# apache/incubator-predictionio

Measured on NVIDIA H100. Metric: ALS iterations/sec, higher is better.
Workload: dtype f32

## Files before the change

### incubator-predictionio_b200/csrc/als_pair_kernel.cuh

```cuda
#pragma once
#include <cuda_fp16.h>
#include <cuda_runtime.h>
#include <stdint.h>

#include "als_kernels.cuh"
#include "als_lockstep.cuh"

namespace pio {
namespace pr {

constexpr int KP = 64;
constexpr int CH = 8;
constexpr int RSTR = KP;
constexpr int NSTAGE = 4;
constexpr int STAGE = CH * RSTR;
constexpr int NTILE = 20;
using LL = LsLayout<KP>;
constexpr int SLOT_STRIDE = LL::STRIDE;
constexpr int VSTR = 80;
constexpr int PART_FLOATS = LL::SIZE + KP;
static_assert(NSTAGE * STAGE <= SLOT_STRIDE, "the staging ring lives in the second slot");
static_assert(NSTAGE % 2 == 0, "a loop step consumes two stages");
constexpr int W_BVEC = 2 * SLOT_STRIDE;
constexpr int W_COL = W_BVEC + 2 * VSTR;
// ... 137 lines not shown
#pragma unroll
    for (int i = 0; i < 4; ++i) {
#pragma unroll
      for (int e = 0; e < 2; ++e) {
        const int q = 2 * i + e;
        const int c0 = xo[q & 3] + 32 * (q >> 2), c4 = 4 * RSTR + xo[q & 3] + 32 * (1 - (q >> 2));
        const float a0 = XA[c0], a4 = XA[c4], b0 = XB[c0], b4 = XB[c4];
        pb[i][e] = fmaf(wb[0], a0, pb[i][e]);
        pb[i][e] = fmaf(wb[1], a4, pb[i][e]);
        pb[i][e] = fmaf(wb[2], b0, pb[i][e]);
        pb[i][e] = fmaf(wb[3], b4, pb[i][e]);
        split2(__fmul_rn(a0, sc[0]), __fmul_rn(a4, sc[1]), hi[i][e], lo[i][e]);
        split2(__fmul_rn(b0, sc[2]), __fmul_rn(b4, sc[3]), hi[i][e + 2], lo[i][e + 2]);
      }
    }
#pragma unroll
    for (int j = 0; j < 8; ++j) {
      const int bi = j >> 1, be = j & 1;
      const uint64_t bh = pack2(hi[bi][be], hi[bi][be + 2]), bl = pack2(lo[bi][be], lo[bi][be + 2]);
#pragma unroll
      for (int i = bi; i < 4; ++i) {
        const int tile = i * (i + 1) + j;
        float d[4];
        mma_f16_zp(d, lo[i], bh);
        mma_f16_p(d, hi[i], bl);
        mma_f16_p(d, hi[i], bh);
        acc[tile][0] += d[0];
        acc[tile][1] += d[1];
        acc[tile][2] += d[2];
        acc[tile][3] += d[3];
      }
    }
  }
  cp_async_wait<0>();
  __syncwarp();

#pragma unroll
  for (int i = 0; i < 4; ++i)
#pragma unroll
    for (int e = 0; e < 2; ++e) {
      float v = pb[i][e];
      v += __shfl_xor_sync(0xffffffffu, v, 1);
      v += __shfl_xor_sync(0xffffffffu, v, 2);
      if (t == 0) bv[16 * i + 8 * e + g] = v;
    }
  {
    const float* yl = yty ? yty + g * KP + 2 * t : nullptr;
    int tile = 0;
#pragma unroll
    for (int i = 0; i < 4; ++i) {
#pragma unroll
      for (int j = 0; j <= 2 * i + 1; ++j, ++tile) {
        const int cb = j >> 1;
        const int cc = 8 * (j & 1) + 2 * t;
        float d0 = acc[tile][0] * unscale, d1 = acc[tile][1] * unscale;
        float d2 = acc[tile][2] * unscale, d3 = acc[tile][3] * unscale;
        if (yl) {
          const float2 y0 = __ldg(reinterpret_cast<const float2*>(yl + 16 * i * KP + 8 * j));
          const float2 y1 = __ldg(reinterpret_cast<const float2*>(yl + (16 * i + 8) * KP + 8 * j));
          d0 += y0.x; d1 += y0.y;
          d2 += y1.x; d3 += y1.y;
        }
        if (cb < i) {
          *reinterpret_cast<float2*>(slot + LL::offd(i, cb, g, cc)) = make_float2(d0, d1);
          *reinterpret_cast<float2*>(slot + LL::offd(i, cb, g + 8, cc)) = make_float2(d2, d3);
        } else {
          if (cc <= g) slot[LL::diag(i, g, cc)] = d0;
          if (cc + 1 <= g) slot[LL::diag(i, g, cc + 1)] = d1;
          if (cc <= g + 8) slot[LL::diag(i, g + 8, cc)] = d2;
          if (cc + 1 <= g + 8) slot[LL::diag(i, g + 8, cc + 1)] = d3;
        }
      }
    }
  }
  __syncwarp();
}

__device__ __forceinline__ void fill_identity(float* slot, float* bv) {
  const int lane = threadIdx.x & 31;
  for (int o = lane; o < LL::SIZE; o += 32) slot[o] = 0.f;
  __syncwarp();
  for (int r = lane; r < KP; r += 32) {
    slot[LL::at(r, r)] = 1.f;
    bv[r] = 0.f;
  }
  __syncwarp();
}

template <bool IMPLICIT, int WARPS>
__global__ void __launch_bounds__(32 * WARPS, 12 / WARPS) als_solve_pair_kernel(const SolveParams p, int n_items) {
  extern __shared__ __align__(16) float smem_all[];
  const int warp = threadIdx.x >> 5;
  float* smem = smem_all + warp * W_FLOATS;
  float* slot0 = smem;
  float* slot1 = smem + SLOT_STRIDE;
  float* ring = slot1;
  float* bvec = smem + W_BVEC;
  float* colbuf = smem + W_COL;
  float* mval = smem + W_MVAL;
  const int lane = threadIdx.x & 31;
  const int grp = lane >> 4;
  const int npairs = (n_items + 1) >> 1;
  const float c1_root_max = IMPLICIT ? sqrtf(p.alpha * __uint_as_float(__ldg(p.absmax + 1))) : 1.f;
  const int e = split_exponent(__uint_as_float(__ldg(p.absmax)) * c1_root_max);
  const float s = pow2f(e), unscale = pow2f(-2 * e);

#pragma unroll 1
  for (int base = blockIdx.x * WARPS; base < npairs; base += gridDim.x * WARPS) {
    const int pair = base + warp;
    int row0 = -1, row1 = -1;
    if (pair < npairs) {
#pragma unroll 1
      for (int h = 0; h < 2; ++h) {
        const int item = 2 * pair + h;
        float* slot = h ? slot1 : slot0;
        float* bv = bvec + h * VSTR;
        if (item >= n_items) {
          fill_identity(slot, bv);
          continue;
        }
        long long beg, end;
        if (p.partial) {
          beg = p.wl_beg[item];
          end = p.wl_end[item];
        } else {
          const int r = p.row_begin + item;
          beg = p.ptr[r];
          end = p.ptr[r + 1];
          if (h) row1 = r;
          else row0 = r;
        }
        accumulate_row<IMPLICIT>(p, beg, end, s, unscale, IMPLICIT && !p.partial ? p.yty : nullptr, ring, mval, slot, bv);
        if (p.partial) {
          float* out = p.partial + (size_t)item * PART_FLOATS;
          for (int o = lane; o < LL::SIZE / 4; o += 32)
            reinterpret_cast<float4*>(out)[o] = reinterpret_cast<const float4*>(slot)[o];
          for (int o = lane; o < KP; o += 32) out[LL::SIZE + o] = bv[o];
          __syncwarp();
        }
      }
    }
    if (p.partial) continue;
    if (WARPS > 1) __syncthreads();
    if (pair < npairs) {
      const int myrow = grp ? row1 : row0;
      const int rr = myrow < 0 ? p.row_begin : myrow;
      chol_lockstep<KP>(grp ? slot1 : slot0, bvec + grp * VSTR, p.lambda * p.nreg[rr], p.k, colbuf + grp * VSTR,
                        p.dst + (size_t)(p.dst_row_offset + rr) * KP, myrow >= 0, p.fail);
      __syncwarp();
    }
  }
}

template <bool IMPLICIT>
__global__ void __launch_bounds__(32, 12) als_finish_pair_kernel(const SolveParams p, const int* __restrict__ row_part_ptr,
                                                                  int n_rows) {
  extern __shared__ __align__(16) float smem[];
  float* bvec = smem + W_BVEC;
  float* colbuf = smem + W_COL;
  const int lane = threadIdx.x & 31;
  const int grp = lane >> 4;
  const int npairs = (n_rows + 1) >> 1;
#pragma unroll 1
  for (int pair = blockIdx.x; pair < npairs; pair += gridDim.x) {
#pragma unroll 1
    for (int h = 0; h < 2; ++h) {
      const int r = 2 * pair + h;
      float* slot = smem + h * SLOT_STRIDE;
      float* bv = bvec + h * VSTR;
      if (r >= n_rows) {
        fill_identity(slot, bv);
        continue;
      }
      const int p0 = row_part_ptr[r], p1 = row_part_ptr[r + 1];
      for (int o = lane; o < PART_FLOATS / 4; o += 32) {
        float4 s = make_float4(0.f, 0.f, 0.f, 0.f);
        for (int q = p0; q < p1; ++q) {
          const float4 v = __ldg(reinterpret_cast<const float4*>(p.partial + (size_t)q * PART_FLOATS) + o);
          s.x += v.x; s.y += v.y; s.z += v.z; s.w += v.w;
        }
        if (o < LL::SIZE / 4) reinterpret_cast<float4*>(slot)[o] = s;
        else reinterpret_cast<float4*>(bv)[o - LL::SIZE / 4] = s;
      }
      __syncwarp();
      if (IMPLICIT) {
        ls_add_yty<KP>(slot, p.yty);
        __syncwarp();
      }
    }
    const int myrow = 2 * pair + grp;
    const bool valid = myrow < n_rows;
    const int rr = valid ? myrow : 0;
    chol_lockstep<KP>(smem + grp * SLOT_STRIDE, bvec + grp * VSTR, p.lambda * p.nreg[rr], p.k, colbuf + grp * VSTR,
                      p.dst + (size_t)(p.dst_row_offset + rr) * KP, valid, p.fail);
    __syncwarp();
  }
}

}
}
```

### incubator-predictionio_b200/csrc/pio_als.cu

```cuda
#include "../../include/pio_als.h"

#include <cuda_runtime.h>
#include <dlfcn.h>
#include <math.h>
#include <nccl.h>
#include <stdarg.h>
#include <stdio.h>
#include <stdlib.h>
#include <string.h>

#include <chrono>
#include <algorithm>
#include <array>
#include <deque>
#include <exception>
#include <map>
#include <memory>
#include <mutex>
#include <string>
#include <type_traits>
#include <vector>

#include "als_kernels.cuh"
#include "als_mma_kernel.cuh"
// ... 196 lines not shown
}
__global__ void extract_csr_kernel(const uint64_t* keys, const uint32_t* pay, const float* rating, long long b,
                                   long long cnt, int bits_col, const int* p2i_col, int* idx, float* val) {
  const long long t = (long long)blockIdx.x * blockDim.x + threadIdx.x;
  if (t >= cnt) return;
  idx[t] = p2i_col[(int)(keys[b + t] & ((1ull << bits_col) - 1ull))];
  val[t] = rating[pay[b + t]];
}
__global__ void local_rows_kernel(const long long* ptr_full, int row0, int R, long long base, const int* inv,
                                  const uint32_t* deg, const uint32_t* npos, int implicit, long long* ptr,
                                  float* nreg, int* counts , int heavy_t) {
  const int r = blockIdx.x * blockDim.x + threadIdx.x;
  if (r > R) return;
  ptr[r] = ptr_full[row0 + r] - base;
  if (r == R) return;
  const int ext = inv[row0 + r];
  float nr = 0.f;
  if (ext >= 0) {
    const uint32_t d = deg[ext];
    nr = implicit ? (float)npos[ext] : (float)d;
    if (d > 0) atomicAdd(&counts[0], 1);
    if (d > (uint32_t)heavy_t) atomicAdd(&counts[1], 1);
  }
  nreg[r] = nr;
}
__global__ void scatter_init_kernel(const float* ext_f, int n, int k, int kp, const int* perm, const uint32_t* deg,
                                    float* F) {
  const long long o = (long long)blockIdx.x * blockDim.x + threadIdx.x;
  if (o >= (long long)n * kp) return;
  const int r = (int)(o / kp), c = (int)(o % kp);
  float v = 0.f;
  if (c < k && deg[r] > 0) v = ext_f[(size_t)r * k + c];
  F[(size_t)perm[r] * kp + c] = v;
}
__device__ __forceinline__ uint64_t splitmix64_dev(uint64_t x) {
  x += 0x9E3779B97F4A7C15ull;
  uint64_t z = x;
  z = (z ^ (z >> 30)) * 0xBF58476D1CE4E5B9ull;
  z = (z ^ (z >> 27)) * 0x94D049BB133111EBull;
  return z ^ (z >> 31);
}
__global__ void hash_init_kernel(int n, int k, int kp, uint64_t seed, int side, const int* perm,
                                 const uint32_t* deg, float* F) {
  const int r = blockIdx.x * blockDim.x + threadIdx.x;
  if (r >= n) return;
  float* row = F + (size_t)perm[r] * kp;
  if (deg[r] == 0) {
    for (int c = 0; c < kp; ++c) row[c] = 0.f;
    return;
  }
  const uint64_t s = seed ^ 0xA5A5A5A55A5A5A5Aull;
  double nrm = 0.0;
  for (int c = 0; c < k; ++c) {
    const uint64_t ctr = ((uint64_t)r * (uint64_t)k + (uint64_t)c) * 2ull + ((uint64_t)side << 62);
    const uint64_t h1 = splitmix64_dev(s ^ ctr), h2 = splitmix64_dev(s ^ (ctr + 1ull));
    const double u1 = ((double)(h1 >> 11) + 1.0) * (1.0 / 9007199254740992.0);
    const double u2 = (double)(h2 >> 11) * (1.0 / 9007199254740992.0);
    const float g = (float)(sqrt(-2.0 * log(u1)) * cos(2.0 * 3.14159265358979323846 * u2));
    row[c] = g;
    nrm += (double)g * (double)g;
  }
  float nf = (float)sqrt(nrm);
  if (nf == 0.f) nf = 1.f;
  for (int c = 0; c < k; ++c) row[c] = row[c] / nf;
  for (int c = k; c < kp; ++c) row[c] = 0.f;
}
__global__ void gather_factors_kernel(const float* F, int n, int k, int kp, const int* perm, float* out) {
  const long long o = (long long)blockIdx.x * blockDim.x + threadIdx.x;
  if (o >= (long long)n * k) return;
  const int r = (int)(o / k), c = (int)(o % k);
  out[o] = F[(size_t)perm[r] * kp + c];
}
__global__ void has_kernel(const uint32_t* deg, int n, uint8_t* has) {
  const int r = blockIdx.x * blockDim.x + threadIdx.x;
  if (r < n) has[r] = deg[r] > 0 ? 1 : 0;
}
__global__ void cand_ext_kernel(const int* inv, const uint32_t* deg, int n_internal, int* out) {
  const int r = blockIdx.x * blockDim.x + threadIdx.x;
  if (r >= n_internal) return;
  const int ext = inv[r];
  out[r] = (ext >= 0 && deg[ext] > 0) ? ext : -1;
}
__global__ void gather_rows_kernel(const float* F, int kp, const int* rows_ext, int n, const int* perm,
                                   const uint32_t* deg, int n_ext, float* out, uint8_t* valid) {
  const int q = blockIdx.x;
  const int r = rows_ext[q];
  const bool ok = r >= 0 && r < n_ext && deg[r] > 0;
  for (int c = threadIdx.x; c < kp; c += blockDim.x) out[(size_t)q * kp + c] = ok ? F[(size_t)perm[r] * kp + c] : 0.f;
  if (threadIdx.x == 0 && valid) valid[q] = ok ? 1 : 0;
  (void)n;
}
struct IdList {
  int v[40];
};
__global__ void gather_rows_ids_kernel(const float* F, int kp, IdList ids, const int* perm, const uint32_t* deg, int n_ext,
                                       float* out, uint8_t* valid) {
  const int q = blockIdx.x;
  const int r = ids.v[q];
  const bool ok = r >= 0 && r < n_ext && deg[r] > 0;
  for (int c = threadIdx.x; c < kp; c += blockDim.x) out[(size_t)q * kp + c] = ok ? F[(size_t)perm[r] * kp + c] : 0.f;
  if (threadIdx.x == 0 && valid) valid[q] = ok ? 1 : 0;
}
__global__ void copy_rows_kernel(const float* src, int kp, const int* rows, float* out) {
  const int v = blockIdx.x;
  for (int c = threadIdx.x; c < kp; c += blockDim.x) out[(size_t)v * kp + c] = src[(size_t)rows[v] * kp + c];
}
__global__ void synth_kernel(int nu, int ni, long long n, uint64_t seed, int implicit, long long start, int* u,
                             int* it, float* r) {
  const long long e = (long long)blockIdx.x * blockDim.x + threadIdx.x;
  if (e >= n) return;
  const uint64_t base = (uint64_t)(start + e) * 4ull;
  const uint64_t h1 = splitmix64_dev(seed ^ (base + 1ull));
  const uint64_t h2 = splitmix64_dev(seed ^ (base + 2ull));
  const uint64_t h3 = splitmix64_dev(seed ^ (base + 3ull));
  u[e] = (int)(h1 % (uint64_t)nu);
  const double uu = (double)(h2 >> 11) * (1.0 / 9007199254740992.0);
  long long item = (long long)floor(__dmul_rn(__dmul_rn((double)ni, uu), uu));
  if (item > ni - 1) item = ni - 1;
  it[e] = (int)item;
  if (implicit) {
    int tz = h3 == 0 ? 64 : __ffsll((long long)h3) - 1;
    if (tz > 9) tz = 9;
    r[e] = (float)(1 + tz);
  } else {
    r[e] = (float)(1 + (int)(h3 % 5ull));
  }
}

struct Side {
  int n = 0;
  int R = 0;
  int n_internal = 0;
  int bits = 1;
  int* perm = nullptr;
  int* inv = nullptr;
  int* rpos = nullptr;
  int* p2i = nullptr;
  uint32_t* deg = nullptr;
  uint32_t* npos = nullptr;
  long long* ptr = nullptr;
  int* idx = nullptr;
  float* val = nullptr;
  long long nnz_local = 0;
  float* nreg = nullptr;
  float* F = nullptr;
  int* cand_ext = nullptr;
  int n_active = 0, n_heavy = 0;
  SidePlan plan;
  long long* part_beg = nullptr;
  long long* part_end = nullptr;
  int* row_part_ptr = nullptr;
  float* partial = nullptr;
  int n_parts = 0;
  std::vector<int> h_row_part_ptr;
};

enum EvKind { EV_SOLVE = 0, EV_GRAM = 1, EV_COMM = 2, EV_SOLVE_USER = 3, EV_NKIND = 4 };
struct EvPair {
  cudaEvent_t a, b;
  int kind;
};

}

using namespace pio;

struct pio_als_handle {
  pio_als_config cfg;
  int KP = 0;
  cudaStream_t stream = nullptr;
  Side U, I;
  float* yty = nullptr;
  double* gram_partial = nullptr;
  double* gram_gsum = nullptr;
  const Side* gram_side = nullptr;
  cudaEvent_t ev_gram = nullptr;
  int gram_blocks = 0;
  int* d_fail = nullptr;
  int* d_counts = nullptr;
  unsigned* d_absmax = nullptr;
  long long* d_timing = nullptr;
  float* d_dbg = nullptr;
  size_t dbg_rows = 0;
  SolveSwitches sw;
  cudaStream_t aux = nullptr, comm_st = nullptr;
  cudaEvent_t ev_start = nullptr, ev_heavy = nullptr, ev_piece[8] = {}, ev_comm = nullptr;
  bool pieces_done = false;
  bool trace_on = false;
  std::chrono::steady_clock::time_point t_prev;
  unsigned char* srv_dev = nullptr;
  size_t srv_dev_cap = 0;
  unsigned char* srv_host = nullptr;
  unsigned char* srv_host_dev = nullptr;
  size_t srv_host_cap = 0;
  unsigned* srv_counter = nullptr;
  unsigned srv_seq = 0;
  bool serve_fused = true;
  bool score_blocked = true;
  bool serve_trace = false;
  float* tc_out = nullptr;
  size_t tc_out_rows = 0;
  bool have_ratings = false, have_init = false, trained = false;
  ncclComm_t comm = nullptr;
  std::string err;
  pio_als_stats st{};
  double phase_ms[8] = {0, 0, 0, 0, 0, 0, 0, 0};
  std::deque<EvPair> ev_pool;
  size_t ev_used = 0;
  std::mutex mu;
  int sm_count = 0;
};

namespace pio {

static int vfail(std::string& sink, int code, const char* fmt, va_list ap) {
  char buf[512];
  vsnprintf(buf, sizeof buf, fmt, ap);
  sink = buf;
  return code;
}
static int fail(pio_als_handle* h, int code, const char* fmt, ...) {
  va_list ap;
  va_start(ap, fmt);
  const int rc = vfail(h ? h->err : g_create_error, code, fmt, ap);
  va_end(ap);
  return rc;
}
static int fail_to(std::string* sink, int code, const char* fmt, ...) {
  va_list ap;
  va_start(ap, fmt);
  const int rc = vfail(*sink, code, fmt, ap);
  va_end(ap);
  return rc;
}
static void tmark(pio_als_handle* h, const char* what) {
  if (!h->trace_on) return;
  cudaStreamSynchronize(h->stream);
  const auto now = std::chrono::steady_clock::now();
  fprintf(stderr, "[pio_als ingest r%d] %-34s %8.3f ms\n", h->cfg.world_rank, what,
          std::chrono::duration<double, std::milli>(now - h->t_prev).count());
  h->t_prev = now;
}
#define CK(h, call)                                                                              \
  do {                                                                                           \
    cudaError_t e_ = (call);                                                                     \
    if (e_ != cudaSuccess)                                                                       \
      return fail(h, PIO_ALS_ERR_CUDA, "%s failed: %s (%s:%d)", #call, cudaGetErrorString(e_), \
                  __FILE__, __LINE__);                                                           \
  } while (0)
#define LAUNCHED(h) (++(h)->st.kernel_launches)

static inline unsigned nblk(long long n, int t) { return (unsigned)((n + t - 1) / t); }

template <class T>
static cudaError_t dalloc(pio_als_handle* h, T** p, size_t n) {
  return cudaMallocAsync((void**)p, (n ? n : 1) * sizeof(T), h->stream);
}
template <class T>
static void dfree(pio_als_handle* h, T*& p) {
  if (p) cudaFreeAsync((void*)p, h->stream);
  p = nullptr;
}

struct Scratch {
  cudaStream_t s;
  std::vector<void*> ptrs;
  explicit Scratch(cudaStream_t s_) : s(s_) {}
  Scratch(const Scratch&) = delete;
  Scratch& operator=(const Scratch&) = delete;
  template <class T>
  cudaError_t alloc(T** p, size_t n) {
    const cudaError_t e = cudaMallocAsync((void**)p, (n ? n : 1) * sizeof(T), s);
    if (e == cudaSuccess) ptrs.push_back((void*)*p);
    return e;
  }
  ~Scratch() {
    for (void* q : ptrs) cudaFreeAsync(q, s);
  }
};

struct CallMem {
  std::vector<cudaStream_t> drain, streams;
  std::vector<cudaEvent_t> events;
  std::vector<void*> dev, pinned;
  CallMem() = default;
  explicit CallMem(cudaStream_t st) : drain{st} {}
  CallMem(const CallMem&) = delete;
  CallMem& operator=(const CallMem&) = delete;
  template <class T>
  cudaError_t device(T** p, size_t n) {
    const size_t bytes = n * sizeof(T);
    const cudaError_t e = cudaMalloc((void**)p, bytes ? bytes : 1);
    if (e == cudaSuccess) dev.push_back((void*)*p);
    return e;
  }
  template <class T>
  cudaError_t host(T** p, size_t n) {
    const size_t bytes = n * sizeof(T);
    const cudaError_t e = cudaHostAlloc((void**)p, bytes ? bytes : 1, cudaHostAllocDefault);
    if (e == cudaSuccess) pinned.push_back((void*)*p);
    return e;
  }
  cudaError_t stream(cudaStream_t* s) {
    const cudaError_t e = cudaStreamCreateWithFlags(s, cudaStreamNonBlocking);
    if (e == cudaSuccess) drain.push_back(*s), streams.push_back(*s);
    return e;
  }
  cudaError_t event(cudaEvent_t* ev) {
    const cudaError_t e = cudaEventCreate(ev);
    if (e == cudaSuccess) events.push_back(*ev);
    return e;
  }
  ~CallMem() {
    for (cudaStream_t s : drain) cudaStreamSynchronize(s);
    for (void* q : dev) cudaFree(q);
    for (void* q : pinned) cudaFreeHost(q);
    for (cudaStream_t s : streams) cudaStreamDestroy(s);
    for (cudaEvent_t e : events) cudaEventDestroy(e);
  }
};

static void free_side(pio_als_handle* h, Side& s, bool keep_factors) {
  dfree(h, s.perm); dfree(h, s.inv); dfree(h, s.rpos); dfree(h, s.p2i); dfree(h, s.deg); dfree(h, s.npos); dfree(h, s.ptr);
  dfree(h, s.idx); dfree(h, s.val); dfree(h, s.nreg); dfree(h, s.cand_ext);
  dfree(h, s.part_beg); dfree(h, s.part_end); dfree(h, s.row_part_ptr); dfree(h, s.partial);
  s.n_parts = 0;
  s.h_row_part_ptr.clear();
  if (!keep_factors) dfree(h, s.F);
}

static EvPair& next_ev(pio_als_handle* h, int kind) {
  if (h->ev_used == h->ev_pool.size()) {
    EvPair p;
    cudaEventCreate(&p.a);
    cudaEventCreate(&p.b);
    p.kind = kind;
    h->ev_pool.push_back(p);
  }
  EvPair& p = h->ev_pool[h->ev_used++];
  p.kind = kind;
  return p;
}

static int build_side(pio_als_handle* h, Side& row, const Side& col, const int* rowext, const int* colext,
                      const float* rating, long long nnz, long long nnz_global) {
  cudaStream_t st = h->stream;
  const int W = h->cfg.world_size, rk = h->cfg.world_rank;
  Scratch tmp(h->stream);
  SortBufs sb;
  for (int i : {0, 1}) {
    CK(h, tmp.alloc(&sb.k[i], (size_t)nnz));
    CK(h, tmp.alloc(&sb.v[i], (size_t)nnz));
  }
  if (nnz > 0) {
    make_keys_int_kernel<<<nblk(nnz, 256), 256, 0, st>>>(rowext, colext, nnz, row.perm, col.rpos, col.bits, sb.keys(),
                                                         sb.vals());
    LAUNCHED(h);
    CK(h, radix_sort_pairs(sb, (size_t)nnz, row.bits + col.bits, st, &h->st.kernel_launches));
  }
  tmark(h, "  side: keys + radix sort");
  const uint64_t* ks = sb.keys();
  const uint32_t* vs = sb.vals();
  long long* ptr_full = nullptr;
  CK(h, tmp.alloc(&ptr_full, (size_t)row.n_internal + 1));
  CK(h, cudaMemsetAsync(ptr_full, 0, sizeof(long long) * ((size_t)row.n_internal + 1), st));
  if (nnz > 0) {
    build_ptr_kernel<<<nblk(nnz, 256), 256, 0, st>>>(ks, nnz, col.bits, row.n_internal, ptr_full);
    LAUNCHED(h);
  }
  long long be[2];
  CK(h, cudaMemcpyAsync(&be[0], ptr_full + (size_t)rk * row.R, sizeof(long long), cudaMemcpyDeviceToHost, st));
  CK(h, cudaMemcpyAsync(&be[1], ptr_full + (size_t)(rk + 1) * row.R, sizeof(long long), cudaMemcpyDeviceToHost, st));
  CK(h, cudaStreamSynchronize(st));
  row.nnz_local = be[1] - be[0];
  if (row.nnz_local >= (1ll << 31))
    return fail(h, PIO_ALS_ERR_ARG, "more than 2^31-1 ratings on one GPU (%lld); use more GPUs", row.nnz_local);
  CK(h, dalloc(h, &row.idx, (size_t)row.nnz_local));
  CK(h, dalloc(h, &row.val, (size_t)row.nnz_local));
  CK(h, dalloc(h, &row.ptr, (size_t)row.R + 1));
  CK(h, dalloc(h, &row.nreg, (size_t)row.R));
  if (row.nnz_local > 0) {
    extract_csr_kernel<<<nblk(row.nnz_local, 256), 256, 0, st>>>(ks, vs, rating, be[0], row.nnz_local, col.bits,
                                                                 col.p2i, row.idx, row.val);
    LAUNCHED(h);
  }
  tmark(h, "  side: ptr + extract csr");
  CK(h, cudaMemsetAsync(h->d_counts, 0, 2 * sizeof(int), st));
  row.plan = plan_side(h->sw, h->KP, row.n, nnz_global);
  local_rows_kernel<<<nblk(row.R + 1, 256), 256, 0, st>>>(ptr_full, rk * row.R, row.R, be[0], row.inv, row.deg,
                                                           row.npos, h->cfg.implicit_prefs, row.ptr, row.nreg,
                                                           h->d_counts, row.plan.heavy_t);
  LAUNCHED(h);
  int counts[2];
  CK(h, cudaMemcpyAsync(counts, h->d_counts, sizeof counts, cudaMemcpyDeviceToHost, st));
  CK(h, cudaStreamSynchronize(st));
  row.n_active = counts[0];
  row.n_heavy = counts[1];
  tmark(h, "  side: local rows");
  if (row.n_heavy > 0) {
    std::vector<long long> hp((size_t)row.n_heavy + 1);
    CK(h, cudaMemcpyAsync(hp.data(), row.ptr, sizeof(long long) * hp.size(), cudaMemcpyDeviceToHost, st));
    CK(h, cudaStreamSynchronize(st));
    std::vector<long long> pb, pe;
    std::vector<int> rpp((size_t)row.n_heavy + 1);
    const int part_len = row.plan.part_len;
    for (int r = 0; r < row.n_heavy; ++r) {
      rpp[r] = (int)pb.size();
      for (long long b = hp[r]; b < hp[r + 1]; b += part_len) {
        pb.push_back(b);
        pe.push_back(b + part_len < hp[r + 1] ? b + part_len : hp[r + 1]);
      }
    }
    rpp[row.n_heavy] = (int)pb.size();
    row.n_parts = (int)pb.size();
    row.h_row_part_ptr = rpp;
    tmark(h, "  side: parts of long rows");
    CK(h, dalloc(h, &row.part_beg, pb.size()));
    CK(h, dalloc(h, &row.part_end, pe.size()));
    CK(h, dalloc(h, &row.row_part_ptr, rpp.size()));
    CK(h, cudaMemcpyAsync(row.part_beg, pb.data(), sizeof(long long) * pb.size(), cudaMemcpyHostToDevice, st));
    CK(h, cudaMemcpyAsync(row.part_end, pe.data(), sizeof(long long) * pe.size(), cudaMemcpyHostToDevice, st));
    CK(h, cudaMemcpyAsync(row.row_part_ptr, rpp.data(), sizeof(int) * rpp.size(), cudaMemcpyHostToDevice, st));
    CK(h, cudaStreamSynchronize(st));
  }
  (void)W;
  return PIO_ALS_OK;
}

static int rank_rows(pio_als_handle* h, Side& s) {
  cudaStream_t st = h->stream;
  Scratch tmp(h->stream);
  SortBufs sb;
  for (int i : {0, 1}) {
    CK(h, tmp.alloc(&sb.k[i], (size_t)s.n));
    CK(h, tmp.alloc(&sb.v[i], (size_t)s.n));
  }
  degree_keys_kernel<<<nblk(s.n, 256), 256, 0, st>>>(s.deg, s.n, sb.keys(), sb.vals());
  LAUNCHED(h);
  CK(h, radix_sort_pairs(sb, (size_t)s.n, 32, st, &h->st.kernel_launches));
  fill_int_kernel<<<nblk(s.n_internal, 256), 256, 0, st>>>(s.inv, s.n_internal, -1);
  LAUNCHED(h);
  assign_internal_kernel<<<nblk(s.n, 256), 256, 0, st>>>(sb.vals(), s.n, h->cfg.world_size, s.R, s.perm, s.inv,
                                                         s.rpos, s.p2i);
  LAUNCHED(h);
  return PIO_ALS_OK;
}

struct XArr {
  const void* in;
  void** out;
  size_t elem;
};
static int exchange_events(pio_als_handle* h, Scratch& keep, SortBufs& sb, long long n, XArr* arrs, int na,
                           long long* n_out) {
  cudaStream_t st = h->stream;
  NcclApi& nc = nccl_api();
  const int W = h->cfg.world_size, me = h->cfg.world_rank;
  Scratch tmp(h->stream);
  if (n > 0) CK(h, radix_sort_pairs(sb, (size_t)n, ceil_log2((uint64_t)W), st, &h->st.kernel_launches));
  const uint64_t* ks = sb.keys();
  const uint32_t* vs = sb.vals();
  long long *d_off = nullptr, *d_cnt = nullptr, *d_all = nullptr;
  CK(h, tmp.alloc(&d_off, (size_t)W + 1));
  CK(h, tmp.alloc(&d_cnt, (size_t)W));
  CK(h, tmp.alloc(&d_all, (size_t)W * W));
  CK(h, cudaMemsetAsync(d_off, 0, sizeof(long long) * (W + 1), st));
  if (n > 0) {
    build_ptr_kernel<<<nblk(n, 256), 256, 0, st>>>(ks, n, 0, W, d_off);
    LAUNCHED(h);
  }
  std::vector<long long> off(W + 1), all((size_t)W * W);
  CK(h, cudaMemcpyAsync(off.data(), d_off, sizeof(long long) * (W + 1), cudaMemcpyDeviceToHost, st));
  CK(h, cudaStreamSynchronize(st));
  std::vector<long long> cnt(W);
  for (int p = 0; p < W; ++p) cnt[p] = off[p + 1] - off[p];
  CK(h, cudaMemcpyAsync(d_cnt, cnt.data(), sizeof(long long) * W, cudaMemcpyHostToDevice, st));
  if (nc.AllGather(d_cnt, d_all, (size_t)W, ncclInt64, h->comm, st) != ncclSuccess)
    return fail(h, PIO_ALS_ERR_COMM, "ncclAllGather (exchange counts) failed");
  CK(h, cudaMemcpyAsync(all.data(), d_all, sizeof(long long) * W * W, cudaMemcpyDeviceToHost, st));
  CK(h, cudaStreamSynchronize(st));
  tmark(h, "  exchange: sort by rank + counts");
  std::vector<long long> roff(W + 1, 0);
  for (int src = 0; src < W; ++src) roff[src + 1] = roff[src] + all[(size_t)src * W + me];
  const long long nrecv = roff[W];
  if (nrecv >= (1ll << 32)) return fail(h, PIO_ALS_ERR_ARG, "more than 2^32-1 events on one rank after the exchange");
  std::vector<unsigned char*> sendbufs(na, nullptr), recvbufs(na, nullptr);
  for (int a = 0; a < na; ++a) {
    if (!arrs[a].in) { *arrs[a].out = nullptr; continue; }
    CK(h, tmp.alloc(&sendbufs[a], (size_t)(n > 0 ? n : 1) * arrs[a].elem));
    CK(h, keep.alloc(&recvbufs[a], (size_t)(nrecv > 0 ? nrecv : 1) * arrs[a].elem));
    if (n > 0) {
      if (arrs[a].elem == 4)
        gather_by_index_kernel<uint32_t><<<nblk(n, 256), 256, 0, st>>>((const uint32_t*)arrs[a].in, vs, n, (uint32_t*)sendbufs[a]);
      else
        gather_by_index_kernel<uint64_t><<<nblk(n, 256), 256, 0, st>>>((const uint64_t*)arrs[a].in, vs, n, (uint64_t*)sendbufs[a]);
      LAUNCHED(h);
    }
    *arrs[a].out = recvbufs[a];
  }
  if (nc.GroupStart() != ncclSuccess) return fail(h, PIO_ALS_ERR_COMM, "ncclGroupStart failed");
  for (int a = 0; a < na; ++a) {
    if (!arrs[a].in) continue;
    for (int p = 0; p < W; ++p) {
      const long long sc = cnt[p], rc_ = all[(size_t)p * W + me];
      if (sc > 0 && nc.Send(sendbufs[a] + (size_t)off[p] * arrs[a].elem, (size_t)sc * arrs[a].elem, ncclInt8, p, h->comm, st) != ncclSuccess)
        return fail(h, PIO_ALS_ERR_COMM, "ncclSend failed");
      if (rc_ > 0 && nc.Recv(recvbufs[a] + (size_t)roff[p] * arrs[a].elem, (size_t)rc_ * arrs[a].elem, ncclInt8, p, h->comm, st) != ncclSuccess)
        return fail(h, PIO_ALS_ERR_COMM, "ncclRecv failed");
    }
  }
  if (nc.GroupEnd() != ncclSuccess) return fail(h, PIO_ALS_ERR_COMM, "ncclGroupEnd failed");
  CK(h, cudaStreamSynchronize(st));
  tmark(h, "  exchange: gather + send/recv");
  *n_out = nrecv;
  return PIO_ALS_OK;
}

static int ingest_device(pio_als_handle* h, const int* d_user, const int* d_item, const float* d_rating,
                         long long nnz, int dedup, const long long* d_ts, bool sharded) {
  cudaStream_t st = h->stream;
  const int W = h->cfg.world_size;
  sharded = sharded && W > 1;
  if (nnz <= 0 && !sharded)
    return fail(h, PIO_ALS_ERR_ARG, "ratings cannot be empty (the templates require(!ratings.take(1).isEmpty))");
  if (nnz < 0) return fail(h, PIO_ALS_ERR_ARG, "nnz < 0");
  if (nnz >= (1ll << 32)) return fail(h, PIO_ALS_ERR_ARG, "nnz must be < 2^32 per call");
  if (dedup < 0 || dedup > 2) return fail(h, PIO_ALS_ERR_ARG, "bad dedup_mode %d", dedup);
  free_side(h, h->U, true);
  free_side(h, h->I, true);
  h->have_ratings = false;
  Side& U = h->U;
  Side& I = h->I;
  U.n = h->cfg.n_users;
  I.n = h->cfg.n_items;
  U.R = (U.n + W - 1) / W;
  I.R = (I.n + W - 1) / W;
  U.n_internal = U.R * W;
  I.n_internal = I.R * W;
  U.bits = ceil_log2((uint64_t)U.n_internal);
  I.bits = ceil_log2((uint64_t)I.n_internal);

  h->trace_on = getenv("PIO_ALS_INGEST_TRACE") != nullptr;
  h->t_prev = std::chrono::steady_clock::now();
  auto mark = [&](const char* what) { tmark(h, what); };
  CK(h, cudaMemsetAsync(h->d_fail, 0, sizeof(int), st));
  if (nnz > 0) {
    validate_coo_kernel<<<nblk(nnz, 256), 256, 0, st>>>(d_user, d_item, nnz, U.n, I.n, h->d_fail);
    LAUNCHED(h);
  }
  int bad = 0;
  CK(h, cudaMemcpyAsync(&bad, h->d_fail, sizeof(int), cudaMemcpyDeviceToHost, st));
  CK(h, cudaStreamSynchronize(st));
  if (bad) return fail(h, PIO_ALS_ERR_ARG, "%d ratings have a user/item index out of range", bad);

  mark("validate");
  Scratch tmp(h->stream);
  const int* su = d_user;
  const int* si = d_item;
  const float* sr = d_rating;
  const long long* sts = d_ts;
  long long ns = nnz;
  if (sharded && dedup != PIO_ALS_DEDUP_NONE) {
    Scratch xs(h->stream);
    SortBufs sb;
    for (int i : {0, 1}) {
      CK(h, xs.alloc(&sb.k[i], (size_t)nnz));
      CK(h, xs.alloc(&sb.v[i], (size_t)nnz));
    }
    if (nnz > 0) {
      dest_mod_kernel<<<nblk(nnz, 256), 256, 0, st>>>(d_user, nnz, W, sb.keys(), sb.vals());
      LAUNCHED(h);
    }
    void *xu = nullptr, *xi = nullptr, *xr = nullptr, *xt = nullptr;
    XArr arrs[4] = {{d_user, &xu, 4}, {d_item, &xi, 4}, {d_rating, &xr, 4},
                    {dedup == PIO_ALS_DEDUP_KEEP_LAST ? (const void*)d_ts : nullptr, &xt, 8}};
// ... 174 lines not shown
static_assert(TC_ROWS_PER_CTA == tc::Api::kPerCta && TC_SOLVE_ROWS_PER_CTA == tc::Api::kSolveWarps, "tc::Api");
static_assert(LS128_FINISH_ROWS_PER_CTA == FIN128_WARPS, "FIN128_WARPS");
static_assert(PART % Cfg16::CH == 0 && PART % Cfg32::CH == 0 && PART % Cfg64::CH == 0 && PART % Cfg128::CH == 0 &&
              PART % mm::CH == 0 && PART % tc::STAGE_RATINGS == 0, "PART");
static_assert(PAIR_PART % pr::CH == 0 && pr::CH == 8, "PAIR_PART and PIO_ALS_PART round to multiples of pr::CH");

static int ensure_dyn_smem(pio_als_handle* h, const void* kernel, size_t bytes, bool carveout = false) {
  struct Rec {
    size_t bytes = 0;
    bool carveout = false;
  };
  static std::mutex mu;
  static std::map<std::pair<const void*, int>, Rec> recs;
  std::lock_guard<std::mutex> lk(mu);
  Rec& r = recs[std::make_pair(kernel, h->cfg.device)];
  if (r.bytes < bytes) {
    CK(h, cudaFuncSetAttribute(kernel, cudaFuncAttributeMaxDynamicSharedMemorySize, (int)bytes));
    r.bytes = bytes;
  }
  if (carveout && !r.carveout) {
    CK(h, cudaFuncSetAttribute(kernel, cudaFuncAttributePreferredSharedMemoryCarveout, 100));
    r.carveout = true;
  }
  return PIO_ALS_OK;
}

template <typename... KArgs, typename... Args>
static int solve_launch(pio_als_handle* h, void (*kernel)(KArgs...), int grid, int block, size_t smem, bool carveout,
                        cudaStream_t st, Args... args) {
  const int rc = ensure_dyn_smem(h, (const void*)kernel, smem, carveout);
  if (rc) return rc;
  kernel<<<grid, block, smem, st>>>(args...);
  LAUNCHED(h);
  ++h->st.solve_launches;
  CK(h, cudaGetLastError());
  return PIO_ALS_OK;
}

static void (*pair_kernel(int warps, bool imp))(const SolveParams, int) {
  switch (warps) {
    case 1: return imp ? pr::als_solve_pair_kernel<true, 1> : pr::als_solve_pair_kernel<false, 1>;
    case 2: return imp ? pr::als_solve_pair_kernel<true, 2> : pr::als_solve_pair_kernel<false, 2>;
    case 6: return imp ? pr::als_solve_pair_kernel<true, 6> : pr::als_solve_pair_kernel<false, 6>;
    case 12: return imp ? pr::als_solve_pair_kernel<true, 12> : pr::als_solve_pair_kernel<false, 12>;
    default: return imp ? pr::als_solve_pair_kernel<true, 4> : pr::als_solve_pair_kernel<false, 4>;
  }
}

static int tc_buffers(pio_als_handle* h, const Side& dst, tc::Api::Params* tp) {
  using A = tc::Api;
  tp->dbg = nullptr;
  tp->timing = nullptr;
  tp->out = nullptr;
  tp->out_row0 = 0;
  if (h->sw.tc_timing) {
    if (!h->d_timing) CK(h, cudaMalloc((void**)&h->d_timing, (size_t)h->sm_count * 16 * 8 * sizeof(long long)));
    cudaMemsetAsync(h->d_timing, 0, (size_t)h->sm_count * 16 * 8 * sizeof(long long), h->stream);
    tp->timing = h->d_timing;
  }
  if (h->sw.tc_debug) {
    if (h->dbg_rows < (size_t)dst.R) {
      if (h->d_dbg) cudaFree(h->d_dbg);
      CK(h, cudaMalloc((void**)&h->d_dbg, (size_t)dst.R * A::kRowFloats * sizeof(float)));
      h->dbg_rows = dst.R;
    }
    cudaMemsetAsync(h->d_dbg, 0, (size_t)dst.R * A::kRowFloats * sizeof(float), h->stream);
    tp->dbg = h->d_dbg;
  }
  if (h->sw.tc_split) {
    const int nlight = dst.n_active - dst.n_heavy;
    const size_t need = (size_t)(nlight < TC_TILE_ROWS ? nlight : TC_TILE_ROWS);
    if (h->tc_out_rows < need) {
      if (h->tc_out) cudaFree(h->tc_out);
      h->tc_out = nullptr;
      h->tc_out_rows = 0;
      CK(h, cudaMalloc((void**)&h->tc_out, need * A::kRowFloats * sizeof(float)));
      h->tc_out_rows = need;
    }
  }
  return PIO_ALS_OK;
}

template <class Cfg>
static int launch_solve_cfg(pio_als_handle* h, Side& dst, const Side& src) {
  SolveParams p0;
  p0.ptr = dst.ptr;
  p0.idx = dst.idx;
  p0.val = dst.val;
  p0.src = src.F;
  p0.dst = dst.F;
  p0.yty = h->yty;
  p0.nreg = dst.nreg;
  p0.fail = h->d_fail;
  p0.lambda = (float)h->cfg.lambda;
  p0.alpha = (float)h->cfg.alpha;
  p0.k = h->cfg.rank;
  p0.dst_row_offset = h->cfg.world_rank * dst.R;
  p0.absmax = h->d_absmax;
  p0.wl_beg = nullptr;
  p0.wl_end = nullptr;
  p0.partial = nullptr;
  p0.n_items = 0;
  const bool imp = h->cfg.implicit_prefs != 0;
  const SolvePlan plan = plan_half_step(h->sw, dst.plan, Cfg::KP, h->sm_count, dst.R, dst.n_active, dst.n_heavy,
                                        dst.n_parts, dst.h_row_part_ptr);
  const bool pair = dst.plan.kernel == SOLVE_PAIR;
  if (pair) cudaEventRecord(h->ev_start, h->stream);
  if (plan.partial_parts > 0 && !dst.partial) {
    const size_t floats = pair ? pr::PART_FLOATS : Cfg::PART_FLOATS;
    CK(h, cudaMallocAsync((void**)&dst.partial, sizeof(float) * (size_t)plan.partial_parts * floats, h->stream));
    if (pair) cudaEventRecord(h->ev_start, h->stream);
  }
  if (plan.n_aux > 0) cudaStreamWaitEvent(h->aux, h->ev_start, 0);
  size_t next_piece = 0;
  auto record_events = [&](int issued) {
    if (pair && issued == plan.n_aux) cudaEventRecord(h->ev_heavy, h->aux);
    for (; next_piece < plan.piece_after.size() && plan.piece_after[next_piece] == issued; ++next_piece)
      cudaEventRecord(h->ev_piece[next_piece], h->stream);
  };
  record_events(0);
  const int warps = h->sw.pair_warps;
  tc::Api::Params tp;
  bool tc_ready = false;
  for (size_t i = 0; i < plan.launches.size(); ++i) {
    const SolveLaunch& L = plan.launches[i];
    const cudaStream_t st = L.aux ? h->aux : h->stream;
    const int nrows = L.row_end - L.row_begin;
    SolveParams p = p0;
    if (L.stage == STAGE_ROWS || L.stage == STAGE_TC_SOLVE) {
      p.row_begin = L.row_begin;
      p.row_end = L.row_end;
    } else {
      p.wl_beg = dst.part_beg + L.wl_off;
      p.wl_end = dst.part_end + L.wl_off;
      p.partial = dst.partial;
      p.n_items = L.wl_count;
      p.row_begin = 0;
      p.row_end = dst.n_heavy;
    }
    auto fp32 = [&] {
      return solve_launch(h, imp ? als_solve_kernel<Cfg, true> : als_solve_kernel<Cfg, false>, L.grid, Cfg::NT,
                          Cfg::smem_bytes(), false, st, p);
    };
    auto pair_items = [&](int n_items) {
      return solve_launch(h, pair_kernel(warps, imp), L.grid, 32 * warps, pr::smem_bytes(warps), true, st, p, n_items);
    };
    int rc = PIO_ALS_OK;
    switch (L.stage) {
      case STAGE_PARTS:
        rc = pair ? pair_items(L.wl_count) : fp32();
        break;
      case STAGE_FINISH:
        rc = pair ? solve_launch(h, imp ? pr::als_finish_pair_kernel<true> : pr::als_finish_pair_kernel<false>, L.grid,
                                 32, pr::smem_bytes(1), true, st, p, dst.row_part_ptr, nrows)
                  : solve_launch(h, imp ? als_finish_kernel<Cfg, true> : als_finish_kernel<Cfg, false>, L.grid,
                                 32 * FINISH_ROWS_PER_CTA, sizeof(float) * 4 * (Cfg::SLOT + 4 * Cfg::KP), false, st, p,
                                 dst.row_part_ptr, nrows);
        break;
      case STAGE_LS128_TILE:
        rc = fp32();
        break;
      case STAGE_LS128_FINISH:
        rc = solve_launch(h, imp ? als_finish_ls128_kernel<true> : als_finish_ls128_kernel<false>, L.grid,
                          32 * FIN128_WARPS, sizeof(float) * (size_t)FIN128_FLOATS * FIN128_WARPS, false, st, p,
                          dst.row_part_ptr, L.row_begin, nrows, L.wl_off);
        break;
      case STAGE_ROWS:
        switch (dst.plan.kernel) {
          case SOLVE_PAIR:
            rc = pair_items(nrows);
            break;
          case SOLVE_MMA:
            rc = solve_launch(h, imp ? mm::als_solve_mma_kernel<true> : mm::als_solve_mma_kernel<false>, L.grid, mm::NT,
                              mm::SMEM_BYTES, false, st, p);
            break;
          case SOLVE_WGMMA:
            if (!tc_ready) {
              rc = tc_buffers(h, dst, &tp);
              if (rc) return rc;
              tc_ready = true;
            }
            tp.sp = p;
            tp.out = h->sw.tc_split ? h->tc_out : nullptr;
            tp.out_row0 = L.row_begin;
            rc = solve_launch(h, tc::Api::kernel(imp), L.grid, tc::Api::kThreads, tc::Api::kSmem, false, st, tp);
            break;
          default:
            rc = fp32();
        }
        break;
      case STAGE_TC_SOLVE:
        rc = solve_launch(h, tc::Api::solver(imp), L.grid, 32 * tc::Api::kSolveWarps, tc::Api::kSolveSmem, false, st, p,
                          (const float*)h->tc_out, L.row_begin);
        break;
    }
    if (rc) return rc;
    record_events((int)i + 1);
  }
  if (pair) {
    cudaStreamWaitEvent(h->stream, h->ev_heavy, 0);
    h->pieces_done = true;
  }
  return PIO_ALS_OK;
}

static int launch_solve(pio_als_handle* h, Side& dst, const Side& src) {
  switch (h->KP) {
    case 16: return launch_solve_cfg<Cfg16>(h, dst, src);
    case 32: return launch_solve_cfg<Cfg32>(h, dst, src);
    case 64: return launch_solve_cfg<Cfg64>(h, dst, src);
    default: return launch_solve_cfg<Cfg128>(h, dst, src);
  }
}

static bool gram_sharded(const pio_als_handle* h) { return h->cfg.world_size > 1 && GRAM_GROUPS % h->cfg.world_size == 0; }
static void gram_layout(const pio_als_handle* h, GramMap& m, int& my_groups, int& slot0) {
  const bool shard = gram_sharded(h);
  const int W = shard ? h->cfg.world_size : 1, me = shard ? h->cfg.world_rank : 0;
  my_groups = GRAM_GROUPS / W;
  slot0 = me * my_groups;
  int seen[GRAM_GROUPS] = {}, mine = 0;
  for (int g = 0; g < GRAM_GROUPS; ++g) {
    const int blk = g / W, pos = g % W;
    const int owner = (blk & 1) ? (W - 1 - pos) : pos;
    m.slot_of[g] = owner * my_groups + seen[owner]++;
    if (owner == me) m.cls[mine++] = g;
  }
  for (int lg = mine; lg < GRAM_GROUPS; ++lg) m.cls[lg] = 0;
}
static int gram_local(pio_als_handle* h, const Side& s) {
  GramMap m;
  int my_groups, slot0;
  gram_layout(h, m, my_groups, slot0);
  const int bpg = h->gram_blocks / GRAM_GROUPS, n = h->KP * h->KP, grid = my_groups * bpg;
  switch (h->KP) {
    case 16: gram_partial_kernel<16><<<grid, GRAM_THREADS, 0, h->stream>>>(s.F, s.p2i, s.n, h->gram_partial, slot0, bpg, m); break;
    case 32: gram_partial_kernel<32><<<grid, GRAM_THREADS, 0, h->stream>>>(s.F, s.p2i, s.n, h->gram_partial, slot0, bpg, m); break;
    case 64: gram_partial_kernel<64><<<grid, GRAM_THREADS, 0, h->stream>>>(s.F, s.p2i, s.n, h->gram_partial, slot0, bpg, m); break;
    default: gram_partial_kernel<128><<<grid, GRAM_THREADS, 0, h->stream>>>(s.F, s.p2i, s.n, h->gram_partial, slot0, bpg, m); break;
  }
  LAUNCHED(h);
  gram_group_kernel<<<dim3(nblk(n, 128), my_groups), 128, 0, h->stream>>>(h->gram_partial, bpg, n, slot0, h->gram_gsum);
  LAUNCHED(h);
  CK(h, cudaGetLastError());
  return PIO_ALS_OK;
}
static int gram_exchange(pio_als_handle* h, cudaStream_t comm_stream) {
  if (!gram_sharded(h)) return PIO_ALS_OK;
  const int n = h->KP * h->KP, my_groups = GRAM_GROUPS / h->cfg.world_size;
  const size_t cnt = (size_t)my_groups * n;
  if (nccl_api().AllGather(h->gram_gsum + (size_t)h->cfg.world_rank * cnt, h->gram_gsum, cnt, ncclDouble, h->comm, comm_stream) !=
      ncclSuccess)
    return fail(h, PIO_ALS_ERR_COMM, "ncclAllGather (YtY class sums) failed");
  return PIO_ALS_OK;
}
static int gram_reduce(pio_als_handle* h, const Side& s) {
  GramMap m;
  int my_groups, slot0;
  gram_layout(h, m, my_groups, slot0);
  const int n = h->KP * h->KP;
  gram_reduce_kernel<<<nblk(n, 256), 256, 0, h->stream>>>(h->gram_gsum, n, h->yty, m);
  LAUNCHED(h);
  CK(h, cudaGetLastError());
  h->gram_side = &s;
  return PIO_ALS_OK;
}

static int half_step(pio_als_handle* h, Side& dst, const Side& src, bool more) {
  cudaStream_t st = h->stream;
  const bool implicit = h->cfg.implicit_prefs != 0;
  if (implicit && h->gram_side != &src) {
    const EvPair e = next_ev(h, EV_GRAM);
    cudaEventRecord(e.a, st);
    int grc = gram_local(h, src);
    if (!grc) grc = gram_exchange(h, st);
    if (!grc) grc = gram_reduce(h, src);
    if (grc) return grc;
    cudaEventRecord(e.b, st);
  }
  {
    const EvPair e = next_ev(h, &dst == &h->U ? EV_SOLVE_USER : EV_SOLVE);
    cudaEventRecord(e.a, st);
    h->pieces_done = false;
    if (h->gram_side == &dst) h->gram_side = nullptr;
    if (dst.plan.kernel == SOLVE_PAIR) {
      const long long n = (long long)src.n_internal * h->KP;
      CK(h, cudaMemsetAsync(h->d_absmax, 0, sizeof(unsigned), st));
      pr::abs_max_kernel<<<4 * h->sm_count, 256, 0, st>>>(src.F, n, h->d_absmax);
      LAUNCHED(h);
    }
    const int rc = launch_solve(h, dst, src);
    if (rc) return rc;
    cudaEventRecord(e.b, st);
  }
  const bool prep = implicit && more;
  bool gram_pending = false;
  if (h->cfg.world_size > 1) {
    NcclApi& nc = nccl_api();
    const int W = h->cfg.world_size, me = h->cfg.world_rank;
    const EvPair e = next_ev(h, EV_COMM);
    if (h->pieces_done && h->sw.n_pieces > 1) {
      cudaStream_t sc = h->comm_st;
      const int C = h->sw.n_pieces;
      bool first = true;
      for (int c = 0; c < C; ++c) {
        const long long lo = (long long)dst.R * c / C, hi = (long long)dst.R * (c + 1) / C;
        if (hi <= lo) continue;
// ... 6534 lines not shown
```

Measured before the change: 35.33.

## Split pair finish reduction into column slices with last-arriver solve

The finish kernel for heavy-row pairs used to reduce every partial of a row pair inside a single warp, which serializes long part lists. Each pair's reduction is now split into host-precomputed column slices handled by different CTAs. Each slice writes its sums back into the first partial, and the last CTA to arrive, detected through an atomic counter, loads the totals with cp.async and runs the Cholesky solve. Loads are batched four deep per column to expose memory parallelism. The cost is an extra write and read of the summed partials, threadfences and atomics, and a per-pair counter that must be reset on every call.

```diff
diff --git a/incubator-predictionio_b200/csrc/als_pair_kernel.cuh b/incubator-predictionio_b200/csrc/als_pair_kernel.cuh
--- a/incubator-predictionio_b200/csrc/als_pair_kernel.cuh
+++ b/incubator-predictionio_b200/csrc/als_pair_kernel.cuh
@@ -313,43 +313,104 @@
   }
 }
 
+constexpr int PART_COLS = PART_FLOATS / 4;
+constexpr int FINISH_MAX_SLICES = 32;
+constexpr int FINISH_PARTS_PER_SLICE = 16;
+constexpr int FINISH_COLS = 2;
+constexpr int FINISH_LOADS = 4;
+
+__device__ __forceinline__ void sum_parts(const float4* __restrict__ part, const int (&q0)[FINISH_COLS],
+                                          const int (&q1)[FINISH_COLS], const int (&o)[FINISH_COLS],
+                                          float4 (&s)[FINISH_COLS]) {
+  int n = 0;
+#pragma unroll
+  for (int k = 0; k < FINISH_COLS; ++k) {
+    s[k] = make_float4(0.f, 0.f, 0.f, 0.f);
+    n = max(n, q1[k] - q0[k]);
+  }
+#pragma unroll 1
+  for (int j0 = 0; j0 < n; j0 += FINISH_LOADS) {
+    float4 v[FINISH_COLS][FINISH_LOADS];
+#pragma unroll
+    for (int k = 0; k < FINISH_COLS; ++k)
+#pragma unroll
+      for (int j = 0; j < FINISH_LOADS; ++j)
+        v[k][j] = __ldg(part + (size_t)min(q0[k] + j0 + j, max(q1[k] - 1, q0[k])) * PART_COLS + o[k]);
+#pragma unroll
+    for (int k = 0; k < FINISH_COLS; ++k)
+#pragma unroll
+      for (int j = 0; j < FINISH_LOADS; ++j)
+        if (q0[k] + j0 + j < q1[k]) {
+          s[k].x += v[k][j].x; s[k].y += v[k][j].y; s[k].z += v[k][j].z; s[k].w += v[k][j].w;
+        }
+  }
+}
+
 template <bool IMPLICIT>
 __global__ void __launch_bounds__(32, 12) als_finish_pair_kernel(const SolveParams p, const int* __restrict__ row_part_ptr,
-                                                                  int n_rows) {
+                                                                  const int4* __restrict__ slices, unsigned* count,
+                                                                  int n_slices, int n_rows) {
   extern __shared__ __align__(16) float smem[];
   float* bvec = smem + W_BVEC;
   float* colbuf = smem + W_COL;
   const int lane = threadIdx.x & 31;
   const int grp = lane >> 4;
-  const int npairs = (n_rows + 1) >> 1;
-#pragma unroll 1
-  for (int pair = blockIdx.x; pair < npairs; pair += gridDim.x) {
+  float4* part = reinterpret_cast<float4*>(p.partial);
+#pragma unroll 1
+  for (int w = blockIdx.x; w < n_slices; w += gridDim.x) {
+    const int4 sl = __ldg(slices + w);
+    const int pair = sl.x;
+    const int rows = n_rows - 2 * pair < 2 ? 1 : 2;
+    const int r0 = 2 * pair;
+    const int q00 = __ldg(row_part_ptr + r0), q01 = __ldg(row_part_ptr + r0 + 1);
+    const int q11 = rows == 2 ? __ldg(row_part_ptr + r0 + 2) : q01;
+    const bool single = sl.w == 1;
+#pragma unroll 1
+    for (int c0 = sl.y + lane; c0 < sl.z; c0 += 32 * FINISH_COLS) {
+      int h[FINISH_COLS], o[FINISH_COLS], q0[FINISH_COLS], q1[FINISH_COLS];
+#pragma unroll
+      for (int k = 0; k < FINISH_COLS; ++k) {
+        const int c = c0 + 32 * k < sl.z ? c0 + 32 * k : c0;
+        h[k] = c >= PART_COLS;
+        o[k] = c - h[k] * PART_COLS;
+        q0[k] = h[k] ? q01 : q00;
+        q1[k] = c0 + 32 * k >= sl.z ? q0[k] : h[k] ? q11 : q01;
+      }
+      float4 s[FINISH_COLS];
+      sum_parts(part, q0, q1, o, s);
+#pragma unroll
+      for (int k = 0; k < FINISH_COLS; ++k) {
+        if (c0 + 32 * k >= sl.z) break;
+        if (!single) part[(size_t)q0[k] * PART_COLS + o[k]] = s[k];
+        else if (o[k] < LL::SIZE / 4) reinterpret_cast<float4*>(smem + h[k] * SLOT_STRIDE)[o[k]] = s[k];
+        else reinterpret_cast<float4*>(bvec + h[k] * VSTR)[o[k] - LL::SIZE / 4] = s[k];
+      }
+    }
+    if (!single) {
+      __threadfence();
+      __syncwarp();
+      unsigned last = 0;
+      if (lane == 0) last = atomicAdd(count + pair, 1u) == (unsigned)sl.w - 1;
+      if (!__shfl_sync(0xffffffffu, last, 0)) continue;
+      __threadfence();
+#pragma unroll 1
+      for (int h = 0; h < rows; ++h) {
+        const float4* sum = part + (size_t)(h ? q01 : q00) * PART_COLS;
+        for (int o = lane; o < PART_COLS; o += 32)
+          cp_async16(o < LL::SIZE / 4 ? smem + h * SLOT_STRIDE + 4 * o : bvec + h * VSTR + 4 * (o - LL::SIZE / 4), sum + o);
+      }
+      cp_async_commit();
+      cp_async_wait<0>();
+      if (lane == 0) count[pair] = 0;
+    }
+    __syncwarp();
 #pragma unroll 1
     for (int h = 0; h < 2; ++h) {
-      const int r = 2 * pair + h;
-      float* slot = smem + h * SLOT_STRIDE;
-      float* bv = bvec + h * VSTR;
-      if (r >= n_rows) {
-        fill_identity(slot, bv);
-        continue;
-      }
-      const int p0 = row_part_ptr[r], p1 = row_part_ptr[r + 1];
-      for (int o = lane; o < PART_FLOATS / 4; o += 32) {
-        float4 s = make_float4(0.f, 0.f, 0.f, 0.f);
-        for (int q = p0; q < p1; ++q) {
-          const float4 v = __ldg(reinterpret_cast<const float4*>(p.partial + (size_t)q * PART_FLOATS) + o);
-          s.x += v.x; s.y += v.y; s.z += v.z; s.w += v.w;
-        }
-        if (o < LL::SIZE / 4) reinterpret_cast<float4*>(slot)[o] = s;
-        else reinterpret_cast<float4*>(bv)[o - LL::SIZE / 4] = s;
-      }
+      if (h >= rows) fill_identity(smem + h * SLOT_STRIDE, bvec + h * VSTR);
+      else if (IMPLICIT) ls_add_yty<KP>(smem + h * SLOT_STRIDE, p.yty);
       __syncwarp();
-      if (IMPLICIT) {
-        ls_add_yty<KP>(slot, p.yty);
-        __syncwarp();
-      }
-    }
-    const int myrow = 2 * pair + grp;
+    }
+    const int myrow = r0 + grp;
     const bool valid = myrow < n_rows;
     const int rr = valid ? myrow : 0;
     chol_lockstep<KP>(smem + grp * SLOT_STRIDE, bvec + grp * VSTR, p.lambda * p.nreg[rr], p.k, colbuf + grp * VSTR,
diff --git a/incubator-predictionio_b200/csrc/pio_als.cu b/incubator-predictionio_b200/csrc/pio_als.cu
--- a/incubator-predictionio_b200/csrc/pio_als.cu
+++ b/incubator-predictionio_b200/csrc/pio_als.cu
@@ -372,6 +372,9 @@
   int* row_part_ptr = nullptr;
   float* partial = nullptr;
   int n_parts = 0;
+  int4* fin_slices = nullptr;
+  unsigned* fin_count = nullptr;
+  int n_fin_slices = 0;
   std::vector<int> h_row_part_ptr;
 };
 
@@ -544,7 +547,9 @@
   dfree(h, s.perm); dfree(h, s.inv); dfree(h, s.rpos); dfree(h, s.p2i); dfree(h, s.deg); dfree(h, s.npos); dfree(h, s.ptr);
   dfree(h, s.idx); dfree(h, s.val); dfree(h, s.nreg); dfree(h, s.cand_ext);
   dfree(h, s.part_beg); dfree(h, s.part_end); dfree(h, s.row_part_ptr); dfree(h, s.partial);
+  dfree(h, s.fin_slices); dfree(h, s.fin_count);
   s.n_parts = 0;
+  s.n_fin_slices = 0;
   s.h_row_part_ptr.clear();
   if (!keep_factors) dfree(h, s.F);
 }
@@ -560,6 +565,24 @@
   EvPair& p = h->ev_pool[h->ev_used++];
   p.kind = kind;
   return p;
+}
+
+static std::vector<int4> finish_slices(const std::vector<int>& rpp) {
+  const int n_heavy = (int)rpp.size() - 1;
+  const long long C = pr::PART_COLS;
+  std::vector<int4> out;
+  for (int j = 0; 2 * j < n_heavy; ++j) {
+    const long long p0 = rpp[2 * j + 1] - rpp[2 * j];
+    const long long p1 = 2 * j + 1 < n_heavy ? rpp[2 * j + 2] - rpp[2 * j + 1] : 0;
+    const long long per = pr::FINISH_PARTS_PER_SLICE;
+    const int S = (int)std::min<long long>(pr::FINISH_MAX_SLICES, std::max<long long>(1, (p0 + p1 + per - 1) / per));
+    auto column_at = [&](long long w) {
+      return (int)(w <= p0 * C ? (w + p0 - 1) / p0 : C + (w - p0 * C + p1 - 1) / p1);
+    };
+    const long long W = C * (p0 + p1);
+    for (int s = 0; s < S; ++s) out.push_back(make_int4(j, column_at(W * s / S), column_at(W * (s + 1) / S), S));
+  }
+  return out;
 }
 
 static int build_side(pio_als_handle* h, Side& row, const Side& col, const int* rowext, const int* colext,
@@ -641,6 +664,15 @@
     CK(h, cudaMemcpyAsync(row.part_beg, pb.data(), sizeof(long long) * pb.size(), cudaMemcpyHostToDevice, st));
     CK(h, cudaMemcpyAsync(row.part_end, pe.data(), sizeof(long long) * pe.size(), cudaMemcpyHostToDevice, st));
     CK(h, cudaMemcpyAsync(row.row_part_ptr, rpp.data(), sizeof(int) * rpp.size(), cudaMemcpyHostToDevice, st));
+    if (row.plan.kernel == SOLVE_PAIR) {
+      const std::vector<int4> fs = finish_slices(rpp);
+      const int npairs = (row.n_heavy + 1) / 2;
+      row.n_fin_slices = (int)fs.size();
+      CK(h, dalloc(h, &row.fin_slices, fs.size()));
+      CK(h, dalloc(h, &row.fin_count, (size_t)npairs));
+      CK(h, cudaMemcpyAsync(row.fin_slices, fs.data(), sizeof(int4) * fs.size(), cudaMemcpyHostToDevice, st));
+      CK(h, cudaMemsetAsync(row.fin_count, 0, sizeof(unsigned) * npairs, st));
+    }
     CK(h, cudaStreamSynchronize(st));
   }
   (void)W;
@@ -1121,7 +1153,8 @@
         break;
       case STAGE_FINISH:
         rc = pair ? solve_launch(h, imp ? pr::als_finish_pair_kernel<true> : pr::als_finish_pair_kernel<false>, L.grid,
-                                 32, pr::smem_bytes(1), true, st, p, dst.row_part_ptr, nrows)
+                                 32, pr::smem_bytes(1), true, st, p, dst.row_part_ptr, (const int4*)dst.fin_slices,
+                                 dst.fin_count, dst.n_fin_slices, nrows)
                   : solve_launch(h, imp ? als_finish_kernel<Cfg, true> : als_finish_kernel<Cfg, false>, L.grid,
                                  32 * FINISH_ROWS_PER_CTA, sizeof(float) * 4 * (Cfg::SLOT + 4 * Cfg::KP), false, st, p,
                                  dst.row_part_ptr, nrows);
```

New measurement: 35.90 (median of 6 runs). 1.02x the previous value.
